# bacpop/ska.rust

Measured on AMD Instinct MI355X. Metric: genomes/sec ska build+align, 1 000x5 Mbp k=31; bit-exact vs CPU, higher is better.
Workload: dtype u64

## Files before the change

ska.rust_amd/csrc/skx_api.cpp:

```cpp
#include "skx_internal.h"
#include <algorithm>
#include <atomic>
#include <chrono>
#include <cmath>
#include <condition_variable>
#include <deque>
#include <cstdarg>
#include <cstddef>
#include <cstdio>
#include <cstring>
#include <map>
#include <memory>
#include <mutex>
#include <numeric>
#include <unordered_map>
#include <thread>
#include <cerrno>
#include <fcntl.h>
#include <sys/mman.h>
#include <sys/stat.h>
#include <unistd.h>

using namespace skx;

// ... 2482 lines not shown
{
    return skx_guarded([&]() -> int {
    skx_ctx *ctx = a->ctx; hipStream_t st = ctx->stream;
    SKX_HIP(hipSetDevice(ctx->device));
    const size_t S = a->names.size();
    if (a->pieces) {
        skx_pieces *pc = a->pieces;
        if (pc->sample_cells.size() != S) {
            DevBuf<unsigned long long> d; SKX_TRY(d.alloc(S)); SKX_TRY(d.zero(st));
            launch_pieces_cells(pc->data.p, pc->plen.p, pc->cap, (int)S, 1 << pc->logQ, d.p, st);
            std::vector<unsigned long long> h(S);
            SKX_HIP(hipMemcpyAsync(h.data(), d.p, S * 8, hipMemcpyDeviceToHost, st));
            SKX_HIP(hipStreamSynchronize(st));
            pc->sample_cells.assign(h.begin(), h.end());
        }
        for (size_t i = 0; i < S; i++) out[i] = (int64_t)pc->sample_cells[i];
        return SKX_OK;
    }
    if (a->lazy()) { for (size_t i = 0; i < S; i++) out[i] = (int64_t)a->lazy_dict->sample_size[i]; return SKX_OK; }
    DevBuf<unsigned long long> d; SKX_TRY(d.alloc(S)); SKX_TRY(d.zero(st));
    launch_row_nonmissing(a->matrix.p, a->pitch, (int)S, a->n_rows, d.p, st);
    std::vector<unsigned long long> h(S);
    SKX_HIP(hipMemcpyAsync(h.data(), d.p, S * 8, hipMemcpyDeviceToHost, st));
    SKX_HIP(hipStreamSynchronize(st));
    for (size_t i = 0; i < S; i++) out[i] = (int64_t)h[i];
    return SKX_OK;
    });
}

extern "C" int skx_array_pieces_info(skx_array *a, uint64_t *piece_bytes, uint64_t *row_blocks, uint32_t *ranks_per_block)
{
    return skx_guarded([&]() -> int {
    if (!a) { set_error("bad arguments"); return SKX_EINVAL; }
    if (piece_bytes) *piece_bytes = 0;
    if (row_blocks) *row_blocks = 0;
    if (ranks_per_block) *ranks_per_block = 0;
    const skx_pieces *pc = a->pieces;
    if (!pc) return SKX_OK;
    skx_ctx *ctx = a->ctx; hipStream_t st = ctx->stream;
    SKX_HIP(hipSetDevice(ctx->device));
    const uint64_t n = ((uint64_t)1 << pc->logQ) * a->names.size();
    std::vector<uint16_t> h(n);
    SKX_HIP(hipMemcpyAsync(h.data(), pc->plen.p, n * 2, hipMemcpyDeviceToHost, st));
    SKX_HIP(hipStreamSynchronize(st));
    uint64_t b = 0;
    for (uint16_t v : h) b += ((uint64_t)v + 31) / 32 * 16;
    if (piece_bytes) *piece_bytes = b;
    if (row_blocks) *row_blocks = (uint64_t)1 << pc->logQ;
    if (ranks_per_block) *ranks_per_block = pc->cap;
    return SKX_OK;
    });
}

static int array_compact(skx_array *a, DevBuf<uint8_t> &keep, DevBuf<uint64_t> &pos, uint64_t kept, int mask_ambig, bool vcount_from_unambig,
                         bool keys_follow)
{
    skx_ctx *ctx = a->ctx; hipStream_t st = ctx->stream;
    const uint64_t U = a->n_rows; const size_t S = a->names.size();
    const bool filter_ambig_as_missing = vcount_from_unambig;
    if (kept == U && !mask_ambig) {
        if (filter_ambig_as_missing && U) SKX_HIP(hipMemcpyAsync(a->vcount.p, a->unambig.p, U * 4, hipMemcpyDeviceToDevice, st));
        SKX_HIP(hipStreamSynchronize(st));
        return SKX_OK;
    }
    {
        StageTimer t(ctx, &ctx->tm.compact);
        const uint64_t np = pitch_for(kept);
        DevBuf<uint8_t> nm; DevBuf<uint32_t> p2, u2, m2, v2;
        SKX_TRY(nm.alloc((uint64_t)S * np)); SKX_TRY(p2.alloc(kept)); SKX_TRY(u2.alloc(kept)); SKX_TRY(m2.alloc(kept)); SKX_TRY(v2.alloc(kept));
        if (a->pieces) {
            PiecesRowsArgs pa = pieces_args(a);
            pa.out = nm.p; pa.pitch = np; pa.keep = keep.p; pa.kpos = pos.p; pa.mask_ambig = mask_ambig;
            KernelTimer kt(ctx, &ctx->tm.pieces_rows);
            launch_pieces_rows(pa, 1u << a->pieces->logQ, st);
        } else if (a->lazy()) {
            DevBuf<int> d_flag; SKX_TRY(d_flag.alloc(1)); SKX_TRY(d_flag.zero(st));
            AssembleArgs aa = lazy_args(a, d_flag.p);
            aa.matrix = nm.p; aa.pitch = np; aa.keep = keep.p; aa.kpos = pos.p; aa.mask_ambig = mask_ambig;
            { StageTimer t2(ctx, &ctx->tm.assemble); launch_assemble_lazy(a, aa, st, 2); }
            SKX_TRY(lazy_check_missing(a, d_flag));
        } else
            launch_compact_matrix(a->matrix.p, a->pitch, nm.p, np, (int)S, U, keep.p, pos.p, mask_ambig, st);
        launch_compact_u32(a->present.p, p2.p, U, keep.p, pos.p, st);
        launch_compact_u32(a->unambig.p, u2.p, U, keep.p, pos.p, st);
        launch_compact_u32(a->mask.p, m2.p, U, keep.p, pos.p, st);
        launch_compact_u32(filter_ambig_as_missing ? a->unambig.p : a->vcount.p, v2.p, U, keep.p, pos.p, st);
        if (mask_ambig) launch_mask_ambig_stats(m2.p, kept, st);
        if (a->n_kmers == U && keys_follow) {
            if (a->k <= 31) {
                DevBuf<uint64_t> k2; SKX_TRY(k2.alloc(kept));
                launch_compact_u64(a->keys.p, k2.p, U, keep.p, pos.p, st);
                a->keys = std::move(k2);
            } else if (a->host_keys.empty()) {
                DevBuf<uint64_t> k2; SKX_TRY(k2.alloc(kept * 2));
                launch_compact_u128(a->keys.p, k2.p, U, keep.p, pos.p, st);
                a->keys = std::move(k2);
            } else {
                std::vector<uint8_t> hkeep(U);
                SKX_HIP(hipMemcpyAsync(hkeep.data(), keep.p, U, hipMemcpyDeviceToHost, st));
                SKX_HIP(hipStreamSynchronize(st));
                std::vector<skx_key> nk; nk.reserve(kept);
                for (uint64_t i = 0; i < U; i++) if (hkeep[i] == 1) nk.push_back(a->host_keys[i]);
                a->host_keys.swap(nk);
            }
            a->n_kmers = kept;
        }
        SKX_HIP(hipStreamSynchronize(st));
        a->matrix = std::move(nm); a->present = std::move(p2); a->unambig = std::move(u2); a->mask = std::move(m2); a->vcount = std::move(v2);
        a->pitch = np; a->n_rows = kept;
        a->drop_lazy();
    }
    return SKX_OK;
}

extern "C" int skx_array_filter(skx_array *a, uint64_t min_count, int filter_ambig_as_missing, int filter_type, int mask_ambig,
                                int ignore_const_gaps, int update_kmers, int32_t *removed)
{
    return skx_guarded([&]() -> int {
    skx_ctx *ctx = a->ctx; hipStream_t st = ctx->stream;
    SKX_HIP(hipSetDevice(ctx->device));
    const uint64_t U = a->n_rows; const size_t S = a->names.size();
    SKX_TRY(array_lazy_stats(a));
    DevBuf<uint8_t> keep; DevBuf<uint64_t> pos;
    SKX_TRY(keep.alloc(U)); SKX_TRY(pos.alloc(U + 1));
    uint64_t kept = 0, silent = 0;
    {
        StageTimer t(ctx, &ctx->tm.filter);
        FilterArgs fa{a->vcount.p, a->present.p, a->unambig.p, a->mask.p, U, (uint32_t)(a->total_samples ? a->total_samples : S), min_count, filter_ambig_as_missing, filter_type, ignore_const_gaps, keep.p};
        launch_filter_flags(fa, st);
        DevBuf<uint32_t> sc_sums; DevBuf<uint64_t> sc_offs;
        SKX_TRY(sc_sums.alloc(scan_u8_blocks(U))); SKX_TRY(sc_offs.alloc(scan_u8_blocks(U) + 1));
        launch_scan_u8(keep.p, pos.p, U, sc_sums.p, sc_offs.p, st);
        SKX_HIP(hipMemcpyAsync(&kept, pos.p + U, 8, hipMemcpyDeviceToHost, st));
        if (filter_ambig_as_missing) {
            DevBuf<unsigned long long> d_sil; SKX_TRY(d_sil.alloc(1)); SKX_TRY(d_sil.zero(st));
            launch_count_u8(keep.p, U, 2, d_sil.p, st);
            unsigned long long s2 = 0;
            SKX_HIP(hipMemcpyAsync(&s2, d_sil.p, 8, hipMemcpyDeviceToHost, st));
            SKX_HIP(hipStreamSynchronize(st));
            silent = s2;
        }
        SKX_HIP(hipStreamSynchronize(st));
    }
    SKX_TRY(array_compact(a, keep, pos, kept, mask_ambig, filter_ambig_as_missing != 0, update_kmers || filter_ambig_as_missing));
    SKX_HIP(hipGetLastError());
    if (removed) *removed = (int32_t)(U - kept - silent);
    return SKX_OK;
    });
}


static int array_keep_rows(skx_array *a, DevBuf<uint8_t> &keep, uint64_t *removed)
{
    hipStream_t st = a->ctx->stream;
    const uint64_t U = a->n_rows;
    DevBuf<uint64_t> pos; SKX_TRY(pos.alloc(U + 1));
    uint64_t kept = 0;
    DevBuf<uint32_t> sc_sums; DevBuf<uint64_t> sc_offs;
    SKX_TRY(sc_sums.alloc(scan_u8_blocks(U))); SKX_TRY(sc_offs.alloc(scan_u8_blocks(U) + 1));
    launch_scan_u8(keep.p, pos.p, U, sc_sums.p, sc_offs.p, st);
// ... 473 lines not shown
```

ska.rust_amd/csrc/skx_api_io.cpp:

```cpp
#include "skx_internal.h"
#include "../../include/skx_host.h"
#include <algorithm>
#include <atomic>
#include <chrono>
#include <cmath>
#include <cstdio>
#include <cstring>
#include <memory>
#include <numeric>
#include <thread>
#include <unistd.h>
#include <fcntl.h>

using namespace skx;

extern "C" int skx_cov_histogram(skx_ctx *ctx, const char *fastq_fwd, const char *fastq_rev, int k, int rc, uint32_t *hist)
{
    return skx_guarded([&]() -> int {
    if (!ctx || !fastq_fwd || !fastq_rev || !hist) { set_error("bad arguments"); return SKX_EINVAL; }
    SKX_TRY(check_k(k));
    SKX_HIP(hipSetDevice(ctx->device));
    hipStream_t st = ctx->stream;
    HostStream hs[2];
    const char *files[2] = {fastq_fwd, fastq_rev};
// ... 599 lines not shown
            const uint64_t nb = (row_done * S) & ~7ull, left = have_hi - row_done * S;
            if (left) SKX_HIP(hipMemcpyAsync(d_cells[cur ^ 1].p + (row_done * S - nb), d_cells[cur].p + (row_done * S - base_cell), left, hipMemcpyDeviceToDevice, st));
        }
        SKX_HIP(hipStreamSynchronize(st));
        if (kept + gk > cap - 256) {
            const uint64_t ncap = pitch_for(std::max((kept + gk) * 2, cap * 2));
            DevBuf<uint8_t> nm; SKX_TRY(nm.alloc(S * ncap));
            if (kept) SKX_HIP(hipMemcpy2DAsync(nm.p, ncap, a->matrix.p, cap, kept, S, hipMemcpyDeviceToDevice, st));
            SKX_HIP(hipStreamSynchronize(st));
            a->matrix = std::move(nm); cap = ncap;
        }
        if (gk) launch_compact_rm(in, S, nr, keep.p + row_lo, pos.p, a->matrix.p, cap, kept, f->two_stage ? 0 : f->mask_ambig, st);
        kept += gk;
        row_lo = row_done; cur ^= 1;
        g0 = g1;
    }
    {
        const int wr = sf.walk_result();
        if (wr == SKF_NOT_TAKEN) { a->prealloc.reset(); a.reset(); return load_then_filter(ctx, path, f, out, removed, constant); }
        if (wr != SKX_OK) return wr;
    }
    int status = 0, bad = 0;
    SKX_HIP(hipMemcpyAsync(&status, d_status.p, 4, hipMemcpyDeviceToHost, st));
    SKX_HIP(hipMemcpyAsync(&bad, d_bad.p, 4, hipMemcpyDeviceToHost, st));
    SKX_HIP(hipStreamSynchronize(st));
    SKX_HIP(hipGetLastError());
    t_data.stop();
    if (status == 3) { tail.join(); a.reset(); return load_then_filter(ctx, path, f, out, removed, constant); }
    if (status) { set_error(status == 2 ? "skf: checksum mismatch" : "skf: corrupt snappy block"); return SKX_EFORMAT; }
    if (bad) { set_error("variants contain a byte outside -ACGTMRWSYKVHDBN (not supported on the device path)"); return SKX_EUNSUP; }
    tail.join();
    if (tail_rc != SKX_OK) { set_error("%s", tail_err.c_str()); return tail_rc; }
    PhaseTimer t_fin("load.counts_check_statistics");
    DevBuf<uint32_t> d_counts; SKX_TRY(d_counts.alloc(U));
    SKX_HIP(hipMemcpyAsync(d_counts.p, counts.data(), U * 4, hipMemcpyHostToDevice, st));
    if (!(f->filter_ambig_as_missing && !f->two_stage)) {
        SKX_TRY(d_status.zero(st));
        launch_differ_u32(d_counts.p, present.p, U, d_status.p, st);
        int differ = 0;
        SKX_HIP(hipMemcpyAsync(&differ, d_status.p, 4, hipMemcpyDeviceToHost, st));
        SKX_HIP(hipStreamSynchronize(st));
        if (differ) { a.reset(); return load_then_filter(ctx, path, f, out, removed, constant); }
    }
    unsigned long long n_silent = 0, n_const = 0;
    {
        DevBuf<unsigned long long> d_cnt; SKX_TRY(d_cnt.alloc(2)); SKX_TRY(d_cnt.zero(st));
        launch_count_u8(keep.p, U, 2, d_cnt.p, st); launch_count_u8(keep.p, U, 3, d_cnt.p + 1, st);
        unsigned long long h[2] = {0, 0};
        SKX_HIP(hipMemcpyAsync(h, d_cnt.p, 16, hipMemcpyDeviceToHost, st));
        DevBuf<uint64_t> gpos; DevBuf<uint32_t> s2; DevBuf<uint64_t> o2;
        SKX_TRY(gpos.alloc(U + 1)); SKX_TRY(s2.alloc(scan_u8_blocks(U) + 1)); SKX_TRY(o2.alloc(scan_u8_blocks(U) + 2));
        launch_scan_u8(keep.p, gpos.p, U, s2.p, o2.p, st);
        SKX_TRY(a->present.alloc(kept)); SKX_TRY(a->unambig.alloc(kept)); SKX_TRY(a->mask.alloc(kept)); SKX_TRY(a->vcount.alloc(kept));
        launch_compact_u32(present.p, a->present.p, U, keep.p, gpos.p, st);
        launch_compact_u32(unambig.p, a->unambig.p, U, keep.p, gpos.p, st);
        launch_compact_u32(mask.p, a->mask.p, U, keep.p, gpos.p, st);
        launch_compact_u32((f->filter_ambig_as_missing && !f->two_stage) ? unambig.p : d_counts.p, a->vcount.p, U, keep.p, gpos.p, st);
        if (f->mask_ambig && !f->two_stage) launch_mask_ambig_stats(a->mask.p, kept, st);
        SKX_HIP(hipStreamSynchronize(st));
        n_silent = h[0]; n_const = h[1];
    }
    SKX_HIP(hipGetLastError());
    a->k_bits = sf.m.k_bits; a->version = sf.m.version.empty() ? skx_version() : sf.m.version;
    a->n_rows = kept; a->pitch = cap;
    if (removed) *removed = (int64_t)(U - kept - n_silent - n_const);
    if (constant) *constant = (int64_t)n_const;
    rel.t = std::chrono::steady_clock::now(); rel.on = true;
    *out = a.release();
    return SKX_OK;
    });
}
```

ska.rust_amd/csrc/skx_append.hip:

```cpp
#include "skx_device.h"
#include <cstdlib>
#include <type_traits>

namespace skx {

typedef uint32_t u32x4 __attribute__((ext_vector_type(4)));
typedef const u32x4 __attribute__((address_space(1))) *g4_t;

#ifdef SKX_AP_PROF
__device__ unsigned long long g_ap_prof[16];
#define AP_PROF_START unsigned long long tprof = __builtin_readcyclecounter(), tacc[12] = {0, 0, 0, 0, 0, 0, 0, 0, 0, 0, 0, 0}
#define AP_PROF(i) do { const unsigned long long t_ = __builtin_readcyclecounter(); tacc[(i)] += t_ - tprof; tprof = t_; } while (0)
#define AP_PROF_FLUSH() do { for (int i_ = 0; i_ < 12; i_++) if (tacc[i_] && (i_ >= 6 || (threadIdx.x & 63) == 0)) atomicAdd(&g_ap_prof[i_], tacc[i_]); } while (0)
extern "C" void skx_debug_phase_prof(unsigned long long *out, int reset)
{
    unsigned long long h[16];
    (void)hipDeviceSynchronize();
    (void)hipMemcpyFromSymbol(h, HIP_SYMBOL(g_ap_prof), sizeof(h));
    for (int i = 0; i < 16; i++) out[i] = h[i];
    if (reset) { for (auto &x : h) x = 0; (void)hipMemcpyToSymbol(HIP_SYMBOL(g_ap_prof), h, sizeof(h)); }
}
#else
#define AP_PROF_START do { } while (0)
#define AP_PROF(i) do { } while (0)
// ... 594 lines not shown
    for (uint32_t p = threadIdx.x; p < nrows; p += 256) {
        const uint32_t pr = s_pr[p];
        o_present[r0 + p] = pr; o_vcount[r0 + p] = pr;
        o_unambig[r0 + p] = s_un[p]; o_mask[r0 + p] = s_mk[p];
    }
}
void launch_pieces_stats(const uint8_t *pieces, const uint16_t *plen, const uint16_t *perm, const uint32_t *nrank, const uint32_t *ncnt, const uint64_t *roff, uint32_t cap,
                         int n_samples, int n_blocks, uint32_t *present, uint32_t *unambig, uint32_t *mask, uint32_t *vcount, hipStream_t st)
{
    if (n_blocks <= 0) return;
    const unsigned gy = (cap / 32 + 255u) / 256u;
    static const int direct = knob("stats_direct") ? 1 : 0;
    const uint32_t stage = (cap + 63u) / 64u * 64u;
    hipLaunchKernelGGL(pieces_stats_kernel, dim3((unsigned)n_blocks, gy), dim3(256), (size_t)stage * 6, st, pieces, plen, perm, nrank, ncnt, roff, cap, n_samples, present, unambig, mask, vcount,
                       direct, stage);
}
__global__ __launch_bounds__(256) void pieces_cells_kernel(const uint8_t *pieces, const uint16_t *plen, uint32_t cap, int S, unsigned long long *out)
{
    const uint64_t j = blockIdx.x;
    const int lane = threadIdx.x & 63;
    for (int s = blockIdx.y * 4 + (threadIdx.x >> 6); s < S; s += gridDim.y * 4) {
        const uint32_t pl = plen[j * (uint64_t)S + s];
        const uint32_t *src = reinterpret_cast<const uint32_t *>(pieces + (j * (uint64_t)S + s) * (cap / 2));
        uint32_t c = 0;
        for (uint32_t i = lane; i < (pl + 7u) / 8u; i += 64) { const uint32_t x = src[i]; uint32_t t = x | (x >> 1); t |= t >> 2; c += (uint32_t)__popc(t & 0x11111111u); }
#pragma unroll
        for (int dd = 32; dd >= 1; dd >>= 1) c += __shfl_xor(c, dd, 64);
        if (lane == 0 && c) atomicAdd(&out[s], (unsigned long long)c);
    }
}
void launch_pieces_cells(const uint8_t *pieces, const uint16_t *plen, uint32_t cap, int n_samples, int n_blocks, unsigned long long *out, hipStream_t st)
{
    if (n_blocks <= 0 || n_samples <= 0) return;
    unsigned gy = (unsigned)((n_samples + 3) / 4); if (gy > 16) gy = 16;
    hipLaunchKernelGGL(pieces_cells_kernel, dim3((unsigned)n_blocks, gy), dim3(256), 0, st, pieces, plen, cap, n_samples, out);
}
__global__ __launch_bounds__(256) void region_totals_kernel(const uint32_t *raw, int logB, unsigned long long *out)
{
    __shared__ unsigned long long s_sum[256];
    const uint64_t B = 1ull << logB;
    unsigned long long t = 0;
    for (uint64_t b = threadIdx.x; b < B; b += 256) t += raw[(uint64_t)blockIdx.x * B + b];
    s_sum[threadIdx.x] = t;
    __syncthreads();
    for (int d = 128; d >= 1; d >>= 1) { if ((int)threadIdx.x < d) s_sum[threadIdx.x] += s_sum[threadIdx.x + d]; __syncthreads(); }
    if (threadIdx.x == 0) out[blockIdx.x] = s_sum[0];
}
void launch_region_totals(const uint32_t *raw, int n_samples, int logB, unsigned long long *out, hipStream_t st)
{
    if (n_samples > 0) hipLaunchKernelGGL(region_totals_kernel, dim3((unsigned)n_samples), dim3(256), 0, st, raw, logB, out);
}

constexpr int PR_WAVES = 8;
__device__ static inline uint32_t ap_iupac4(uint32_t m)
{
    const uint32_t idx = m & 0x07070707u;
    const uint32_t lo = __builtin_amdgcn_perm(0x48595754u, 0x4D43412Du, idx);
    const uint32_t hi = __builtin_amdgcn_perm(0x4E42444Bu, 0x56535247u, idx);
    const uint32_t sel = ((m >> 3) & 0x01010101u) * 0xFFu;
    return (hi & sel) | (lo & ~sel);
}
template <bool KEPT>
__global__ __launch_bounds__(64 * PR_WAVES) void pieces_rows_kernel(PiecesRowsArgs a)
{
    extern __shared__ __attribute__((aligned(16))) unsigned char s_raw[];
    const uint32_t cap = a.cap;
    uint16_t *s_src = reinterpret_cast<uint16_t *>(s_raw);
    uint32_t *s_piece = reinterpret_cast<uint32_t *>(s_raw + (((size_t)cap + 16) * 2 + 15) / 16 * 16);
    const uint64_t j = (uint64_t)blockIdx.x + a.j_base;
    const uint32_t n = a.ncnt[j];
    if (n == 0) return;
    const uint64_t r0 = a.roff[j];
    const uint64_t k0 = KEPT ? a.kpos[r0] : 0;
    const uint32_t nout = KEPT ? (uint32_t)(a.kpos[r0 + n] - k0) : n;
    if (nout == 0) return;
    const int tid = threadIdx.x, lane = tid & 63, wv = tid >> 6;
    const uint64_t ocol = KEPT ? k0 : r0 - a.col_base;
    const uint32_t shift = (uint32_t)(ocol & 3u);
    const uint32_t ndw = (nout + shift + 3u) / 4u;
    const uint16_t *pj = a.perm + j * (uint64_t)cap;
    const uint32_t nr = a.nrank[j];
    const int S = a.n_samples;
    const int s_lo = blockIdx.y * a.samples_per_wg, s_hi = s_lo + a.samples_per_wg < S ? s_lo + a.samples_per_wg : S;
    uint32_t *pc = s_piece + (size_t)wv * (cap / 8 + 4);
    const unsigned char *pcb = reinterpret_cast<const unsigned char *>(pc);
    const uint32_t nrw = (nr + 7u) / 8u;
    if (lane < 4) pc[cap / 8 + lane] = 0u;
    for (uint32_t t0 = 0; t0 < nout + shift; t0 += cap) {
        for (uint32_t i = tid; i < cap + 16u; i += blockDim.x) s_src[i] = (uint16_t)cap;
        __syncthreads();
        for (uint32_t r = tid; r < nr; r += blockDim.x) {
            const uint32_t p = pj[r];
            if (p == 0xFFFFu || p >= n) continue;
            uint32_t sc;
            if (!KEPT) sc = shift + p;
            else if (a.keep[r0 + p] == 1) sc = shift + (uint32_t)(a.kpos[r0 + p] - k0);
            else continue;
            if (sc >= t0 && sc < t0 + cap) s_src[sc - t0] = (uint16_t)r;
        }
        __syncthreads();
        const uint32_t v_lo = t0 / 4u, v_hi = (t0 + cap) / 4u < ndw ? (t0 + cap) / 4u : ndw;
        for (int s = s_lo + wv; s < s_hi; s += PR_WAVES) {
            const uint32_t pl = a.plen[j * (uint64_t)S + s];
            const uint32_t plw = (pl + 7u) / 8u;
            const uint32_t *src = reinterpret_cast<const uint32_t *>(a.pieces + (j * (uint64_t)S + s) * (cap / 2));
            {
                const uint4 *src4 = reinterpret_cast<const uint4 *>(src);
                uint4 *pc4 = reinterpret_cast<uint4 *>(pc);
                for (uint32_t i = lane; i < (nrw + 3u) / 4u; i += 64) {
                    uint4 x = 4u * i < plw ? src4[i] : make_uint4(0u, 0u, 0u, 0u);
                    if (4u * i + 1u >= plw) x.y = 0u;
                    if (4u * i + 2u >= plw) x.z = 0u;
                    if (4u * i + 3u >= plw) x.w = 0u;
                    pc4[i] = x;
                }
            }
            __builtin_amdgcn_wave_barrier();
            unsigned char *dst = a.out + (uint64_t)s * a.pitch + (ocol - shift);
            for (uint32_t v = v_lo + lane; v < v_hi; v += 64) {
                const uint2 rr = *reinterpret_cast<const uint2 *>(s_src + 4u * (v - v_lo));
                const uint32_t ra = rr.x & 0xFFFFu, rb = rr.x >> 16, rc = rr.y & 0xFFFFu, rd = rr.y >> 16;
                const uint32_t na = ((uint32_t)pcb[ra >> 1] >> ((ra & 1u) * 4u)) & 15u, nb = ((uint32_t)pcb[rb >> 1] >> ((rb & 1u) * 4u)) & 15u;
                const uint32_t nc = ((uint32_t)pcb[rc >> 1] >> ((rc & 1u) * 4u)) & 15u, nd = ((uint32_t)pcb[rd >> 1] >> ((rd & 1u) * 4u)) & 15u;
                uint32_t m = na | (nb << 8) | (nc << 16) | (nd << 24);
                uint32_t word = ap_iupac4(m);
                if (a.mask_ambig) {
                    const uint32_t y = m & (m - ((m | (m >> 1) | (m >> 2) | (m >> 3)) & 0x01010101u));
                    const uint32_t amb = ((y | (y >> 1) | (y >> 2) | (y >> 3)) & 0x01010101u) * 0xFFu;
                    word = (word & ~amb) | (0x4E4E4E4Eu & amb);
                }
                const bool head = v == 0 && shift != 0, tail = v == ndw - 1 && ((nout + shift) & 3u) != 0;
                if (!head && !tail) *reinterpret_cast<uint32_t *>(dst + 4u * v) = word;
                else {
#pragma unroll
                    for (int b = 0; b < 4; b++) { const int c = (int)(4u * v + b) - (int)shift; if (c >= 0 && (uint32_t)c < nout) dst[4u * v + b] = (unsigned char)(word >> (8 * b)); }
                }
            }
            __builtin_amdgcn_wave_barrier();
        }
        __syncthreads();
    }
}
void launch_pieces_rows(const PiecesRowsArgs &a, uint32_t n_blocks, hipStream_t st)
{
    if (!n_blocks || a.n_samples <= 0) return;
    PiecesRowsArgs b = a;
    int spw = a.n_samples;
    while (spw > PR_WAVES * 4 && (uint64_t)n_blocks * ((a.n_samples + spw - 1) / spw) < 8192) spw = (spw + 1) / 2;
    b.samples_per_wg = spw;
    const unsigned gy = (unsigned)((a.n_samples + spw - 1) / spw);
    const size_t lds = (((size_t)a.cap + 16) * 2 + 15) / 16 * 16 + (size_t)PR_WAVES * (a.cap / 8 + 4) * 4;
    if (a.keep) {
        (void)hipFuncSetAttribute((const void *)pieces_rows_kernel<true>, hipFuncAttributeMaxDynamicSharedMemorySize, (int)lds);
        hipLaunchKernelGGL(pieces_rows_kernel<true>, dim3(n_blocks, gy), dim3(64 * PR_WAVES), lds, st, b);
    } else {
        (void)hipFuncSetAttribute((const void *)pieces_rows_kernel<false>, hipFuncAttributeMaxDynamicSharedMemorySize, (int)lds);
        hipLaunchKernelGGL(pieces_rows_kernel<false>, dim3(n_blocks, gy), dim3(64 * PR_WAVES), lds, st, b);
    }
}

}

#include "skx_append_wide.inc"
```

ska.rust_amd/csrc/skx_device.h:

```cpp
#pragma once
#include <hip/hip_runtime.h>
#include <stdint.h>

namespace skx {

long knob(const char *name, long absent = 0);
int extract_tile_bases(int logB);
constexpr int MAX_LOGB = 13;
constexpr uint64_t EMPTY64 = ~0ull;

struct HashParams {
    int bits;
    int hb;
    uint32_t hmask;
    uint32_t c[4];
};
HashParams make_hash_params(int k);
__host__ __device__ inline uint32_t hround(uint32_t v, uint32_t c, int hb) { return (v * c) >> (32 - hb); }
__host__ __device__ inline void hmix_halves(uint32_t &L, uint32_t &R, const HashParams &p)
{
    L ^= hround(R, p.c[0], p.hb); R ^= hround(L, p.c[1], p.hb);
}
__host__ __device__ inline uint64_t hmix(uint64_t x, const HashParams &p)
{
// ... 85 lines not shown
    uint64_t pitch;
    uint32_t *col_present;
    uint32_t *col_unambig;
    uint32_t *col_mask;
    uint32_t max_rows;
    int *missing;
    uint32_t j_base = 0;
    uint64_t col_base = 0;
    const uint8_t *keep = nullptr; const uint64_t *kpos = nullptr;
    int mask_ambig = 0;
};
void launch_assemble(const AssembleArgs &a, hipStream_t st, int mode = 0, uint32_t n_blocks = 0);
bool union_side_ok(const DictView &d, int logN, uint32_t stride);
void launch_union_side(const DictView &d, int logN, uint64_t *stage, uint32_t stride, uint32_t *ncnt, uint32_t table_slots, int *overflow,
                       uint16_t *side, uint16_t *perm, hipStream_t st);
void launch_assemble_side(const AssembleArgs &a, const uint16_t *side, const uint16_t *perm, hipStream_t st, bool wide = false);
void launch_compose_perm(const uint64_t *l_stage, uint32_t l_stride, const uint32_t *l_ncnt, const uint16_t *l_perm, int l_logN, const uint64_t *g_stage,
                         uint32_t g_stride, const uint32_t *g_ncnt, const uint64_t *g_roff, int g_logN, int bits, uint16_t *g_perm, uint32_t *g_n,
                         uint64_t *g_base, uint32_t *g_max, int *bad, hipStream_t st);
void launch_union_side_wide(const DictView &d, int logN, u128 *stage, uint32_t stride, uint32_t *ncnt, uint32_t table_slots, int *overflow,
                            uint16_t *side, uint16_t *perm, hipStream_t st);

constexpr uint32_t APPEND_MAX_CAP = 6016, APPEND_MAX_SLOTS = 8192;
struct AppendArgs {
    const uint64_t *words; const uint64_t *off; const uint32_t *raw;
    int n_samples, logB, bits, logQ;
    uint32_t nslots, cap;
    uint8_t *pieces; uint16_t *plen; uint16_t *perm; uint32_t *nrank;
    uint64_t *stage; uint32_t stride; uint32_t *ncnt;
    unsigned long long *probe;
    int *overflow;
    uint32_t rounds = 1;
    int *bar = nullptr;
};
bool append_ok(int bits, int logB, int logQ, uint32_t region_cap, uint32_t nslots, uint32_t cap);
void launch_append(const AppendArgs &a, uint32_t region_cap, hipStream_t st);
void launch_append_probe(const AppendArgs &a, uint32_t region_cap, unsigned blocks, hipStream_t st);
constexpr uint32_t APPEND_WIDE_MAX_CAP = 3072, APPEND_WIDE_MAX_SLOTS = 4096;
bool append_wide_ok(int bits, int logB, int logQ, uint32_t nslots, uint32_t cap);
void launch_append_wide(const AppendArgs &a, hipStream_t st);
void launch_append_wide_probe(const AppendArgs &a, unsigned blocks, hipStream_t st);
void launch_pieces_stats(const uint8_t *pieces, const uint16_t *plen, const uint16_t *perm, const uint32_t *nrank, const uint32_t *ncnt, const uint64_t *roff, uint32_t cap,
                         int n_samples, int n_blocks, uint32_t *present, uint32_t *unambig, uint32_t *mask, uint32_t *vcount, hipStream_t st);
void launch_pieces_cells(const uint8_t *pieces, const uint16_t *plen, uint32_t cap, int n_samples, int n_blocks, unsigned long long *out, hipStream_t st);
void launch_region_totals(const uint32_t *raw, int n_samples, int logB, unsigned long long *out, hipStream_t st);
struct PiecesRowsArgs {
    const uint8_t *pieces; const uint16_t *plen; const uint16_t *perm; const uint32_t *nrank; uint32_t cap; int n_samples;
    const uint32_t *ncnt; const uint64_t *roff;
    uint8_t *out; uint64_t pitch;
    uint32_t j_base = 0; uint64_t col_base = 0;
    const uint8_t *keep = nullptr; const uint64_t *kpos = nullptr;
    int mask_ambig = 0;
    int samples_per_wg = 0;
};
void launch_pieces_rows(const PiecesRowsArgs &a, uint32_t n_blocks, hipStream_t st);

void launch_gather_keys(const uint64_t *stage, uint32_t stride, const uint32_t *ncnt, const uint64_t *roff, int n_sub,
                        uint64_t *out, int unhash, HashParams hp, hipStream_t st);
void launch_hash_keys(const uint64_t *keys, uint64_t *words, uint64_t n, HashParams hp, hipStream_t st);
void launch_keys_cbor(const uint64_t *words, uint64_t n, HashParams hp, uint8_t *out, int *short_key, hipStream_t st);
void launch_unhash_dict(const uint64_t *words, uint64_t n, uint64_t *keys, uint8_t *bases, HashParams hp, hipStream_t st);

void launch_col_stats(const uint8_t *matrix, uint64_t pitch, int n_samples, uint64_t n_cols, uint32_t *present,
                      uint32_t *unambig, uint32_t *mask, int *bad_byte, hipStream_t st);
struct FilterArgs {
    const uint32_t *vcount, *present, *unambig, *mask; uint64_t n_cols; uint32_t n_samples;
    uint64_t min_count; int ambig_as_missing, filter_type, ignore_const_gaps;
    uint8_t *keep;
    int two_stage = 0;
};
void launch_filter_flags(const FilterArgs &a, hipStream_t st);
void launch_row_stats_rm(const uint8_t *cells, uint64_t S, uint64_t nr, uint32_t *present, uint32_t *unambig, uint32_t *mask, int *bad_byte, hipStream_t st);
void launch_compact_rm(const uint8_t *cells, uint64_t S, uint64_t nr, const uint8_t *keep, const uint64_t *pos, uint8_t *out, uint64_t pitch,
                       uint64_t col0, int mask_ambig, hipStream_t st);
uint64_t scan_u8_blocks(uint64_t n);
void launch_scan_u8(const uint8_t *flags, uint64_t *pos, uint64_t n, uint32_t *sums, uint64_t *offs, hipStream_t st);
void launch_compact_matrix(const uint8_t *in, uint64_t in_pitch, uint8_t *out, uint64_t out_pitch, int n_samples,
                           uint64_t n_cols, const uint8_t *keep, const uint64_t *pos, int mask_ambig, hipStream_t st);
void launch_compact_u32(const uint32_t *in, uint32_t *out, uint64_t n, const uint8_t *keep, const uint64_t *pos, hipStream_t st);
void launch_compact_u64(const uint64_t *in, uint64_t *out, uint64_t n, const uint8_t *keep, const uint64_t *pos, hipStream_t st);
void launch_compact_u128(const uint64_t *in, uint64_t *out, uint64_t n, const uint8_t *keep, const uint64_t *pos, hipStream_t st);
void launch_mask_ambig_stats(uint32_t *mask, uint64_t n, hipStream_t st);
void launch_count_u8(const uint8_t *v, uint64_t n, uint8_t value, unsigned long long *out, hipStream_t st);
void launch_differ_u32(const uint32_t *a, const uint32_t *b, uint64_t n, int *flag, hipStream_t st);
void launch_transpose(const uint8_t *in, uint64_t in_pitch, uint64_t rows, uint64_t cols, uint8_t *out, uint64_t out_pitch,
                      hipStream_t st);
struct SnapChunk { uint64_t src_off, uoff; uint32_t src_len, ulen, crc, compressed; };
constexpr uint32_t SKF_SLOT = 8 + 65536;
int launch_skf_decode_cells(int device, const uint8_t *src, const SnapChunk *chunks, uint32_t n_chunks, uint64_t upos, uint64_t uend,
                            uint8_t *scratch , uint8_t *cells, uint64_t base_cell, int *status, hipStream_t st);
int launch_skf_encode_cells(int device, const uint8_t *cells, uint64_t base_cell, uint64_t upos, uint64_t uoff0, uint32_t n_chunks,
                            uint8_t *slots, uint32_t *sizes, hipStream_t st);
void launch_skf_gather(const uint8_t *slots, const uint32_t *sizes, const uint64_t *off, uint32_t n_chunks, uint8_t *dense, hipStream_t st);
void launch_row_nonmissing(const uint8_t *matrix, uint64_t pitch, int n_samples, uint64_t n_cols, unsigned long long *out,
                           hipStream_t st);

void launch_build_planes(const uint8_t *matrix, uint64_t pitch, int n_samples, uint64_t n_cols, uint64_t *planes, uint64_t wpr, int filt,
                         hipStream_t st);
void launch_keep_bits(const uint8_t *keep, const uint64_t *pos, uint64_t n, uint64_t *keep_bits, uint64_t *gpos, hipStream_t st);
void launch_split_keep(const uint8_t *keep, const uint32_t *col_mask, uint64_t n, uint8_t *clean, uint8_t *dirty, hipStream_t st, int mode = 0);
void launch_split_keep_from_dirty(uint8_t *dirty, uint64_t n, uint8_t *clean, hipStream_t st);
void launch_build_planes_keep(const uint8_t *matrix, uint64_t pitch, int n_samples, uint64_t n_cols, const uint64_t *keep_bits, const uint64_t *gpos,
                              uint64_t *planes, uint64_t wpr, int filt, hipStream_t st, uint32_t *first_group, uint64_t kept);
constexpr int DIST_NCOUNT = 16;
int launch_pair_counts(const uint64_t *planes, int n_samples, uint64_t words_per_row, int filt_ambig,
                       unsigned long long *out, hipStream_t st, int i_lo = 0, int i_hi = 0);

void launch_hist_wide(const ExtractArgs &a, hipStream_t st);
void launch_scatter_wide(const ExtractArgs &a, hipStream_t st);
int extract_tile_bases_wide();
void launch_dedupe_wide(u128 *words, const uint64_t *off, const uint32_t *raw, uint32_t *ucnt, uint64_t n_regions, uint32_t cap,
                        int rem_bits, int *overflow, uint16_t *sidx, int sb, hipStream_t st);
void launch_union_wide(const DictView &d, int logN, u128 *stage, uint32_t stride, uint32_t *ncnt, uint32_t table_slots, int *overflow,
                       hipStream_t st);
void launch_union_probe_wide(const DictView &d, int logP, int probe, uint32_t *cnt, uint32_t table_slots, int *overflow, hipStream_t st);
void launch_assemble_wide(const AssembleArgs &a, hipStream_t st, int mode = 0, uint32_t n_blocks = 0);
void launch_gather_keys_wide(const u128 *stage, uint32_t stride, const uint32_t *ncnt, const uint64_t *roff, int n_sub, u128 *out,
                             hipStream_t st);

uint64_t fasta_parse_tiles(uint64_t len);
#ifdef __HIPCC__
__device__ static inline void planes_bytes16(const uint64_t *groups, uint64_t t, uint64_t len, uint32_t sw[4], uint32_t qw[4])
{
    const uint64_t p0 = t * 16;
    const uint64_t *g = groups + (t >> 2) * 5;
    const int sh = (int)(t & 3) * 16;
    const uint32_t lo = (uint32_t)(g[0] >> sh) & 0xFFFFu, hi = (uint32_t)(g[1] >> sh) & 0xFFFFu, bad = (uint32_t)(g[2] >> sh) & 0xFFFFu,
                   nl = (uint32_t)(g[3] >> sh) & 0xFFFFu, qb = (uint32_t)(g[4] >> sh) & 0xFFFFu;
#pragma unroll
    for (int i = 0; i < 4; i++) {
        uint32_t x = 0, y = 0;
#pragma unroll
// ... 46 lines not shown
```

ska.rust_amd/csrc/skx_device2.inc:

```
namespace skx {

__device__ static inline uint32_t set_code(uint32_t b)
{
    switch (b) {
    case '-': return 0;
    case 'A': return 1;  case 'C': return 2;  case 'M': return 3;  case 'T': return 4;
    case 'W': return 5;  case 'Y': return 6;  case 'H': return 7;  case 'G': return 8;
    case 'R': return 9;  case 'S': return 10; case 'V': return 11; case 'K': return 12;
    case 'D': return 13; case 'B': return 14; case 'N': return 15;
    default: return 0xFF;
    }
}

__global__ __launch_bounds__(256) void col_stats_kernel(const uint8_t *matrix, uint64_t pitch, int n_samples, uint64_t n_cols,
                                                        uint32_t *present, uint32_t *unambig, uint32_t *mask, int *bad_byte)
{
    const uint64_t c0 = ((uint64_t)blockIdx.x * blockDim.x + threadIdx.x) * 4;
    if (c0 >= n_cols) return;
    uint32_t p[4] = {0, 0, 0, 0}, u[4] = {0, 0, 0, 0}, m[4] = {0, 0, 0, 0};
    int bad = 0;
    for (int s = 0; s < n_samples; s++) {
        const uint32_t x = *reinterpret_cast<const uint32_t *>(matrix + (uint64_t)s * pitch + c0);
#pragma unroll
        for (int i = 0; i < 4; i++) {
// ... 65 lines not shown
        const uint32_t kw[4] = {k4.x, k4.y, k4.z, k4.w};
#pragma unroll
        for (int i = 0; i < 16; i++) kf |= (uint32_t)(((kw[i >> 2] >> (8 * (i & 3))) & 0xFFu) == 1u) << i;
    } else if (c < n_cols)
        for (int i = 0; i < 16; i++) kf |= (uint32_t)(c + i < n_cols && keep[c + i] == 1) << i;
    uint32_t total;
    const uint32_t lofs = block_excl_scan(__popc(kf), s_tmp, &total);
    if (total == 0) return;
    const uint64_t cblk = (uint64_t)blockIdx.x * blockDim.x * 16;
    const uint64_t p0 = pos[cblk < n_cols ? cblk : n_cols - 1];
    const uint32_t shift = (uint32_t)(p0 & 15u);
    const uint32_t stride = (4096 + 32 + 15) & ~15u;
    const int s0 = blockIdx.y * CMP_ROWS, s1 = s0 + CMP_ROWS < n_samples ? s0 + CMP_ROWS : n_samples;
    if (kf) {
        const uint8_t *src = in + (uint64_t)s0 * in_pitch + c;
#pragma unroll 2
        for (int s = s0; s < s1; s++, src += in_pitch) {
            const uint4 x4 = *reinterpret_cast<const uint4 *>(src);
            const uint32_t xw[4] = {x4.x, x4.y, x4.z, x4.w};
            unsigned char *d = s_buf + (size_t)(s - s0) * stride + shift + lofs;
            uint32_t o = 0;
#pragma unroll
            for (int i = 0; i < 16; i++)
                if ((kf >> i) & 1u) { const uint8_t b = (uint8_t)(xw[i >> 2] >> (8 * (i & 3))); d[o++] = mask_ambig ? mask_ambig_byte(b) : b; }
        }
    }
    __syncthreads();
    const int lane = threadIdx.x & 63, wv = threadIdx.x >> 6;
    const uint32_t head = (16u - shift) & 15u, h = head < total ? head : total, body = (total - h) / 16u, done = h + body * 16u;
    for (int s = s0 + wv; s < s1; s += 4) {
        const unsigned char *row = s_buf + (size_t)(s - s0) * stride + shift;
        uint8_t *dst = out + (uint64_t)s * out_pitch + p0;
        if ((uint32_t)lane < h) dst[lane] = row[lane];
        for (uint32_t v = lane; v < body; v += 64) *reinterpret_cast<uint4 *>(dst + h + 16u * v) = *reinterpret_cast<const uint4 *>(row + h + 16u * v);
        if (done + lane < total) dst[done + lane] = row[done + lane];
    }
}
void launch_compact_matrix(const uint8_t *in, uint64_t in_pitch, uint8_t *out, uint64_t out_pitch, int n_samples, uint64_t n_cols,
                           const uint8_t *keep, const uint64_t *pos, int mask_ambig, hipStream_t st)
{
    if (!n_cols || !n_samples) return;
    const uint64_t groups = (n_cols + 15) / 16;
    const size_t lds = (size_t)CMP_ROWS * ((4096 + 32 + 15) & ~15u);
    (void)hipFuncSetAttribute((const void *)compact_matrix_kernel, hipFuncAttributeMaxDynamicSharedMemorySize, (int)lds);
    hipLaunchKernelGGL(compact_matrix_kernel, dim3((unsigned)((groups + 255) / 256), (unsigned)((n_samples + CMP_ROWS - 1) / CMP_ROWS)), dim3(256),
                       lds, st, in, in_pitch, out, out_pitch, n_samples, n_cols, keep, pos, mask_ambig);
}
template <typename T>
__global__ void compact_vec_kernel(const T *in, T *out, uint64_t n, const uint8_t *keep, const uint64_t *pos)
{
    for (uint64_t c = (uint64_t)blockIdx.x * blockDim.x + threadIdx.x; c < n; c += (uint64_t)gridDim.x * blockDim.x)
        if (keep[c] == 1) out[pos[c]] = in[c];
}
void launch_compact_u32(const uint32_t *in, uint32_t *out, uint64_t n, const uint8_t *keep, const uint64_t *pos, hipStream_t st)
{
    if (!n) return;
    uint64_t g = (n + 255) / 256; if (g > 8192) g = 8192;
    hipLaunchKernelGGL(compact_vec_kernel<uint32_t>, dim3((unsigned)g), dim3(256), 0, st, in, out, n, keep, pos);
}
void launch_compact_u64(const uint64_t *in, uint64_t *out, uint64_t n, const uint8_t *keep, const uint64_t *pos, hipStream_t st)
{
    if (!n) return;
    uint64_t g = (n + 255) / 256; if (g > 8192) g = 8192;
    hipLaunchKernelGGL(compact_vec_kernel<uint64_t>, dim3((unsigned)g), dim3(256), 0, st, in, out, n, keep, pos);
}
struct alignas(16) pair64 { uint64_t a, b; };
void launch_compact_u128(const uint64_t *in, uint64_t *out, uint64_t n, const uint8_t *keep, const uint64_t *pos, hipStream_t st)
{
    if (!n) return;
    uint64_t g = (n + 255) / 256; if (g > 8192) g = 8192;
    hipLaunchKernelGGL(compact_vec_kernel<pair64>, dim3((unsigned)g), dim3(256), 0, st, (const pair64 *)in, (pair64 *)out, n, keep, pos);
}
__global__ void mask_ambig_stats_kernel(uint32_t *mask, uint64_t n)
{
    const uint64_t c = (uint64_t)blockIdx.x * blockDim.x + threadIdx.x;
    if (c >= n) return;
    const uint32_t acgt = (1u << 1) | (1u << 2) | (1u << 4) | (1u << 8);
    uint32_t m = mask[c];
    if (m & ~acgt) m = (m & acgt) | (1u << 15);
    mask[c] = m;
}
void launch_mask_ambig_stats(uint32_t *mask, uint64_t n, hipStream_t st)
{
    if (!n) return;
    hipLaunchKernelGGL(mask_ambig_stats_kernel, dim3((unsigned)((n + 255) / 256)), dim3(256), 0, st, mask, n);
}

__global__ __launch_bounds__(256) void row_stats_rm_kernel(const uint8_t *cells, uint64_t S, uint64_t nr, uint32_t *present, uint32_t *unambig,
                                                           uint32_t *mask, int *bad_byte)
{
    __shared__ uint8_t s_lut[256];
    s_lut[threadIdx.x] = (uint8_t)set_code(threadIdx.x);
    __syncthreads();
    const int lane = threadIdx.x & 63;
    const uint64_t waves = (uint64_t)gridDim.x * 4;
    for (uint64_t r = (uint64_t)blockIdx.x * 4 + (threadIdx.x >> 6); r < nr; r += waves) {
        const int64_t b = (int64_t)(r * S), e = b + (int64_t)S;
        const int64_t skew = (int64_t)(((uintptr_t)cells + (uintptr_t)b) & 3u);
        uint32_t p = 0, u = 0, m = 0; bool bad = false;
        for (int64_t a = b - skew + 4 * lane; a < e; a += 256) {
            const uint32_t x = *reinterpret_cast<const uint32_t *>(cells + a);
#pragma unroll
            for (int i = 0; i < 4; i++) {
                const int64_t q = a + i;
                if (q < b || q >= e) continue;
                const uint32_t code = s_lut[(x >> (8 * i)) & 0xFFu];
                if (code == 0xFF) { bad = true; continue; }
                if (code) { p++; u += (code & (code - 1)) == 0; m |= 1u << code; }
            }
        }
        for (int d = 32; d; d >>= 1) { p += __shfl_down(p, d, 64); u += __shfl_down(u, d, 64); m |= __shfl_down(m, d, 64); }
// ... 639 lines not shown
```

Before: 29050.

## Fuse per-column stats compaction and trim kept-row piece loads to highest used rank

Four separate compaction launches for present/unambig/mask/vcount are merged into one kernel that reads keep and pos once. In the kept-rows pieces kernel, the keep/kpos lookups are batched four at a time, and a block-wide max of the used row rank limits how many packed piece words each wave loads into LDS. Debug counters and knobs for counting piece loads and forcing full loads are also added. The trade-off is an extra atomic and barrier per tile, plus some unused instrumentation branches.

```diff
diff --git a/ska.rust_amd/csrc/skx_api.cpp b/ska.rust_amd/csrc/skx_api.cpp
--- a/ska.rust_amd/csrc/skx_api.cpp
+++ b/ska.rust_amd/csrc/skx_api.cpp
@@ -2558,6 +2558,7 @@
     });
 }
 
+extern "C" int skx_debug_kept_piece_loads(unsigned long long *out, int reset);
 static int array_compact(skx_array *a, DevBuf<uint8_t> &keep, DevBuf<uint64_t> &pos, uint64_t kept, int mask_ambig, bool vcount_from_unambig,
                          bool keys_follow)
 {
@@ -2587,10 +2588,7 @@
             SKX_TRY(lazy_check_missing(a, d_flag));
         } else
             launch_compact_matrix(a->matrix.p, a->pitch, nm.p, np, (int)S, U, keep.p, pos.p, mask_ambig, st);
-        launch_compact_u32(a->present.p, p2.p, U, keep.p, pos.p, st);
-        launch_compact_u32(a->unambig.p, u2.p, U, keep.p, pos.p, st);
-        launch_compact_u32(a->mask.p, m2.p, U, keep.p, pos.p, st);
-        launch_compact_u32(filter_ambig_as_missing ? a->unambig.p : a->vcount.p, v2.p, U, keep.p, pos.p, st);
+        launch_compact_stats(a->present.p, a->unambig.p, a->mask.p, filter_ambig_as_missing ? a->unambig.p : a->vcount.p, p2.p, u2.p, m2.p, v2.p, U, keep.p, pos.p, st);
         if (mask_ambig) launch_mask_ambig_stats(m2.p, kept, st);
         if (a->n_kmers == U && keys_follow) {
             if (a->k <= 31) {
@@ -2612,6 +2610,11 @@
             a->n_kmers = kept;
         }
         SKX_HIP(hipStreamSynchronize(st));
+        if (a->pieces && getenv("SKX_DEBUG") && knob("kept_count_ranks")) {
+            unsigned long long c[3] = {0, 0, 0};
+            if (skx_debug_kept_piece_loads(c, 0) == 0)
+                fprintf(stderr, "[skx] kept rows: %llu piece loads, %llu column passes, %llu beyond a block's first (counted since the process began)\n", c[0], c[1], c[2]);
+        }
         a->matrix = std::move(nm); a->present = std::move(p2); a->unambig = std::move(u2); a->mask = std::move(m2); a->vcount = std::move(v2);
         a->pitch = np; a->n_rows = kept;
         a->drop_lazy();
diff --git a/ska.rust_amd/csrc/skx_api_io.cpp b/ska.rust_amd/csrc/skx_api_io.cpp
--- a/ska.rust_amd/csrc/skx_api_io.cpp
+++ b/ska.rust_amd/csrc/skx_api_io.cpp
@@ -675,10 +675,8 @@
         SKX_TRY(gpos.alloc(U + 1)); SKX_TRY(s2.alloc(scan_u8_blocks(U) + 1)); SKX_TRY(o2.alloc(scan_u8_blocks(U) + 2));
         launch_scan_u8(keep.p, gpos.p, U, s2.p, o2.p, st);
         SKX_TRY(a->present.alloc(kept)); SKX_TRY(a->unambig.alloc(kept)); SKX_TRY(a->mask.alloc(kept)); SKX_TRY(a->vcount.alloc(kept));
-        launch_compact_u32(present.p, a->present.p, U, keep.p, gpos.p, st);
-        launch_compact_u32(unambig.p, a->unambig.p, U, keep.p, gpos.p, st);
-        launch_compact_u32(mask.p, a->mask.p, U, keep.p, gpos.p, st);
-        launch_compact_u32((f->filter_ambig_as_missing && !f->two_stage) ? unambig.p : d_counts.p, a->vcount.p, U, keep.p, gpos.p, st);
+        launch_compact_stats(present.p, unambig.p, mask.p, (f->filter_ambig_as_missing && !f->two_stage) ? unambig.p : d_counts.p, a->present.p, a->unambig.p, a->mask.p,
+                             a->vcount.p, U, keep.p, gpos.p, st);
         if (f->mask_ambig && !f->two_stage) launch_mask_ambig_stats(a->mask.p, kept, st);
         SKX_HIP(hipStreamSynchronize(st));
         n_silent = h[0]; n_const = h[1];
diff --git a/ska.rust_amd/csrc/skx_append.hip b/ska.rust_amd/csrc/skx_append.hip
--- a/ska.rust_amd/csrc/skx_append.hip
+++ b/ska.rust_amd/csrc/skx_append.hip
@@ -670,6 +670,16 @@
 }
 
 constexpr int PR_WAVES = 8;
+__device__ unsigned long long g_kept_counts[3];
+extern "C" int skx_debug_kept_piece_loads(unsigned long long *out , int reset)
+{
+    unsigned long long h[3] = {0, 0, 0};
+    hipError_t e = hipDeviceSynchronize();
+    if (e == hipSuccess) e = hipMemcpyFromSymbol(h, HIP_SYMBOL(g_kept_counts), sizeof(h));
+    if (e == hipSuccess && out) for (int i = 0; i < 3; i++) out[i] = h[i];
+    if (e == hipSuccess && reset) { for (auto &x : h) x = 0; e = hipMemcpyToSymbol(HIP_SYMBOL(g_kept_counts), h, sizeof(h)); }
+    return (int)e;
+}
 __device__ static inline uint32_t ap_iupac4(uint32_t m)
 {
     const uint32_t idx = m & 0x07070707u;
@@ -678,10 +688,42 @@
     const uint32_t sel = ((m >> 3) & 0x01010101u) * 0xFFu;
     return (hi & sel) | (lo & ~sel);
 }
+__device__ static inline uint4 pr_trim(uint4 x, uint32_t i, uint32_t plw)
+{
+    if (4u * i >= plw) x.x = 0u;
+    if (4u * i + 1u >= plw) x.y = 0u;
+    if (4u * i + 2u >= plw) x.z = 0u;
+    if (4u * i + 3u >= plw) x.w = 0u;
+    return x;
+}
+__device__ static inline void pr_gather(const PiecesRowsArgs &a, const uint16_t *s_src, const unsigned char *pcb, unsigned char *dst, uint32_t v_lo, uint32_t v_hi,
+                                        uint32_t ndw, uint32_t nout, uint32_t shift, int lane)
+{
+    for (uint32_t v = v_lo + lane; v < v_hi; v += 64) {
+        const uint2 rr = *reinterpret_cast<const uint2 *>(s_src + 4u * (v - v_lo));
+        const uint32_t ra = rr.x & 0xFFFFu, rb = rr.x >> 16, rc = rr.y & 0xFFFFu, rd = rr.y >> 16;
+        const uint32_t na = ((uint32_t)pcb[ra >> 1] >> ((ra & 1u) * 4u)) & 15u, nb = ((uint32_t)pcb[rb >> 1] >> ((rb & 1u) * 4u)) & 15u;
+        const uint32_t nc = ((uint32_t)pcb[rc >> 1] >> ((rc & 1u) * 4u)) & 15u, nd = ((uint32_t)pcb[rd >> 1] >> ((rd & 1u) * 4u)) & 15u;
+        uint32_t m = na | (nb << 8) | (nc << 16) | (nd << 24);
+        uint32_t word = ap_iupac4(m);
+        if (a.mask_ambig) {
+            const uint32_t y = m & (m - ((m | (m >> 1) | (m >> 2) | (m >> 3)) & 0x01010101u));
+            const uint32_t amb = ((y | (y >> 1) | (y >> 2) | (y >> 3)) & 0x01010101u) * 0xFFu;
+            word = (word & ~amb) | (0x4E4E4E4Eu & amb);
+        }
+        const bool head = v == 0 && shift != 0, tail = v == ndw - 1 && ((nout + shift) & 3u) != 0;
+        if (!head && !tail) *reinterpret_cast<uint32_t *>(dst + 4u * v) = word;
+        else {
+#pragma unroll
+            for (int b = 0; b < 4; b++) { const int c = (int)(4u * v + b) - (int)shift; if (c >= 0 && (uint32_t)c < nout) dst[4u * v + b] = (unsigned char)(word >> (8 * b)); }
+        }
+    }
+}
 template <bool KEPT>
 __global__ __launch_bounds__(64 * PR_WAVES) void pieces_rows_kernel(PiecesRowsArgs a)
 {
     extern __shared__ __attribute__((aligned(16))) unsigned char s_raw[];
+    __shared__ uint32_t s_rmax;
     const uint32_t cap = a.cap;
     uint16_t *s_src = reinterpret_cast<uint16_t *>(s_raw);
     uint32_t *s_piece = reinterpret_cast<uint32_t *>(s_raw + (((size_t)cap + 16) * 2 + 15) / 16 * 16);
@@ -702,62 +744,63 @@
     const int s_lo = blockIdx.y * a.samples_per_wg, s_hi = s_lo + a.samples_per_wg < S ? s_lo + a.samples_per_wg : S;
     uint32_t *pc = s_piece + (size_t)wv * (cap / 8 + 4);
     const unsigned char *pcb = reinterpret_cast<const unsigned char *>(pc);
-    const uint32_t nrw = (nr + 7u) / 8u;
     if (lane < 4) pc[cap / 8 + lane] = 0u;
+    unsigned long long n_loads = 0;
     for (uint32_t t0 = 0; t0 < nout + shift; t0 += cap) {
         for (uint32_t i = tid; i < cap + 16u; i += blockDim.x) s_src[i] = (uint16_t)cap;
+        if (KEPT && tid == 0) s_rmax = 0u;
         __syncthreads();
-        for (uint32_t r = tid; r < nr; r += blockDim.x) {
-            const uint32_t p = pj[r];
-            if (p == 0xFFFFu || p >= n) continue;
-            uint32_t sc;
-            if (!KEPT) sc = shift + p;
-            else if (a.keep[r0 + p] == 1) sc = shift + (uint32_t)(a.kpos[r0 + p] - k0);
-            else continue;
-            if (sc >= t0 && sc < t0 + cap) s_src[sc - t0] = (uint16_t)r;
-        }
-        __syncthreads();
+        uint32_t rmax = nr;
+        if (!KEPT) {
+            for (uint32_t r = tid; r < nr; r += blockDim.x) {
+                const uint32_t p = pj[r];
+                if (p == 0xFFFFu || p >= n) continue;
+                const uint32_t sc = shift + p;
+                if (sc >= t0 && sc < t0 + cap) s_src[sc - t0] = (uint16_t)r;
+            }
+            __syncthreads();
+        } else {
+            uint32_t hi = 0;
+            for (uint32_t rb = tid; rb < nr; rb += 4u * blockDim.x) {
+                uint32_t p[4]; uint8_t kp[4]; uint64_t kq[4];
+#pragma unroll
+                for (int i = 0; i < 4; i++) { const uint32_t r = rb + (uint32_t)i * blockDim.x; p[i] = pj[r < nr ? r : 0u]; if (r >= nr) p[i] = 0xFFFFu; }
+#pragma unroll
+                for (int i = 0; i < 4; i++) { const bool ok = p[i] != 0xFFFFu && p[i] < n; if (!ok) p[i] = 0u; kp[i] = a.keep[r0 + p[i]]; if (!ok) kp[i] = 0; }
+#pragma unroll
+                for (int i = 0; i < 4; i++) kq[i] = a.kpos[r0 + p[i]];
+#pragma unroll
+                for (int i = 0; i < 4; i++) {
+                    if (kp[i] != 1) continue;
+                    const uint32_t r = rb + (uint32_t)i * blockDim.x, sc = shift + (uint32_t)(kq[i] - k0);
+                    if (sc >= t0 && sc < t0 + cap) { s_src[sc - t0] = (uint16_t)r; hi = r + 1u; }
+                }
+            }
+#pragma unroll
+            for (int dd = 32; dd >= 1; dd >>= 1) { const uint32_t o = (uint32_t)__shfl_xor((int)hi, dd, 64); hi = o > hi ? o : hi; }
+            if (lane == 0 && hi) atomicMax(&s_rmax, hi);
+            __syncthreads();
+            if (!a.full_pieces) rmax = s_rmax;
+            if (a.count && tid == 0) { atomicAdd(a.count + 1, 1ull); if (t0) atomicAdd(a.count + 2, 1ull); }
+        }
+        const uint32_t nrw = (rmax + 7u) / 8u;
+        const uint32_t nq = (nrw + 3u) / 4u;
         const uint32_t v_lo = t0 / 4u, v_hi = (t0 + cap) / 4u < ndw ? (t0 + cap) / 4u : ndw;
+        uint4 *pc4 = reinterpret_cast<uint4 *>(pc);
         for (int s = s_lo + wv; s < s_hi; s += PR_WAVES) {
             const uint32_t pl = a.plen[j * (uint64_t)S + s];
             const uint32_t plw = (pl + 7u) / 8u;
-            const uint32_t *src = reinterpret_cast<const uint32_t *>(a.pieces + (j * (uint64_t)S + s) * (cap / 2));
-            {
-                const uint4 *src4 = reinterpret_cast<const uint4 *>(src);
-                uint4 *pc4 = reinterpret_cast<uint4 *>(pc);
-                for (uint32_t i = lane; i < (nrw + 3u) / 4u; i += 64) {
-                    uint4 x = 4u * i < plw ? src4[i] : make_uint4(0u, 0u, 0u, 0u);
-                    if (4u * i + 1u >= plw) x.y = 0u;
-                    if (4u * i + 2u >= plw) x.z = 0u;
-                    if (4u * i + 3u >= plw) x.w = 0u;
-                    pc4[i] = x;
-                }
-            }
+            const uint4 *src4 = reinterpret_cast<const uint4 *>(a.pieces + (j * (uint64_t)S + s) * (cap / 2));
+            for (uint32_t i = lane; i < nq; i += 64)
+                pc4[i] = pr_trim(4u * i < plw ? src4[i] : make_uint4(0u, 0u, 0u, 0u), i, plw);
+            if (KEPT && a.count) n_loads += ((plw < nrw ? plw : nrw) + 3u) / 4u;
             __builtin_amdgcn_wave_barrier();
-            unsigned char *dst = a.out + (uint64_t)s * a.pitch + (ocol - shift);
-            for (uint32_t v = v_lo + lane; v < v_hi; v += 64) {
-                const uint2 rr = *reinterpret_cast<const uint2 *>(s_src + 4u * (v - v_lo));
-                const uint32_t ra = rr.x & 0xFFFFu, rb = rr.x >> 16, rc = rr.y & 0xFFFFu, rd = rr.y >> 16;
-                const uint32_t na = ((uint32_t)pcb[ra >> 1] >> ((ra & 1u) * 4u)) & 15u, nb = ((uint32_t)pcb[rb >> 1] >> ((rb & 1u) * 4u)) & 15u;
-                const uint32_t nc = ((uint32_t)pcb[rc >> 1] >> ((rc & 1u) * 4u)) & 15u, nd = ((uint32_t)pcb[rd >> 1] >> ((rd & 1u) * 4u)) & 15u;
-                uint32_t m = na | (nb << 8) | (nc << 16) | (nd << 24);
-                uint32_t word = ap_iupac4(m);
-                if (a.mask_ambig) {
-                    const uint32_t y = m & (m - ((m | (m >> 1) | (m >> 2) | (m >> 3)) & 0x01010101u));
-                    const uint32_t amb = ((y | (y >> 1) | (y >> 2) | (y >> 3)) & 0x01010101u) * 0xFFu;
-                    word = (word & ~amb) | (0x4E4E4E4Eu & amb);
-                }
-                const bool head = v == 0 && shift != 0, tail = v == ndw - 1 && ((nout + shift) & 3u) != 0;
-                if (!head && !tail) *reinterpret_cast<uint32_t *>(dst + 4u * v) = word;
-                else {
-#pragma unroll
-                    for (int b = 0; b < 4; b++) { const int c = (int)(4u * v + b) - (int)shift; if (c >= 0 && (uint32_t)c < nout) dst[4u * v + b] = (unsigned char)(word >> (8 * b)); }
-                }
-            }
+            pr_gather(a, s_src, pcb, a.out + (uint64_t)s * a.pitch + (ocol - shift), v_lo, v_hi, ndw, nout, shift, lane);
             __builtin_amdgcn_wave_barrier();
         }
         __syncthreads();
     }
+    if (KEPT && a.count && lane == 0 && n_loads) atomicAdd(a.count, n_loads);
 }
 void launch_pieces_rows(const PiecesRowsArgs &a, uint32_t n_blocks, hipStream_t st)
 {
@@ -769,6 +812,12 @@
     const unsigned gy = (unsigned)((a.n_samples + spw - 1) / spw);
     const size_t lds = (((size_t)a.cap + 16) * 2 + 15) / 16 * 16 + (size_t)PR_WAVES * (a.cap / 8 + 4) * 4;
     if (a.keep) {
+        b.full_pieces = knob("kept_full_pieces") ? 1 : 0;
+        b.count = nullptr;
+        if (knob("kept_count_ranks") && hipGetSymbolAddress((void **)&b.count, HIP_SYMBOL(g_kept_counts)) != hipSuccess) {
+            b.count = nullptr;
+            fprintf(stderr, "[skx] kept_count_ranks: no address for the counters, nothing is counted\n");
+        }
         (void)hipFuncSetAttribute((const void *)pieces_rows_kernel<true>, hipFuncAttributeMaxDynamicSharedMemorySize, (int)lds);
         hipLaunchKernelGGL(pieces_rows_kernel<true>, dim3(n_blocks, gy), dim3(64 * PR_WAVES), lds, st, b);
     } else {
diff --git a/ska.rust_amd/csrc/skx_device.h b/ska.rust_amd/csrc/skx_device.h
--- a/ska.rust_amd/csrc/skx_device.h
+++ b/ska.rust_amd/csrc/skx_device.h
@@ -161,6 +161,7 @@
     const uint8_t *keep = nullptr; const uint64_t *kpos = nullptr;
     int mask_ambig = 0;
     int samples_per_wg = 0;
+    int full_pieces = 0; unsigned long long *count = nullptr;
 };
 void launch_pieces_rows(const PiecesRowsArgs &a, uint32_t n_blocks, hipStream_t st);
 
@@ -186,7 +187,8 @@
 void launch_scan_u8(const uint8_t *flags, uint64_t *pos, uint64_t n, uint32_t *sums, uint64_t *offs, hipStream_t st);
 void launch_compact_matrix(const uint8_t *in, uint64_t in_pitch, uint8_t *out, uint64_t out_pitch, int n_samples,
                            uint64_t n_cols, const uint8_t *keep, const uint64_t *pos, int mask_ambig, hipStream_t st);
-void launch_compact_u32(const uint32_t *in, uint32_t *out, uint64_t n, const uint8_t *keep, const uint64_t *pos, hipStream_t st);
+void launch_compact_stats(const uint32_t *in_p, const uint32_t *in_u, const uint32_t *in_m, const uint32_t *in_v, uint32_t *out_p, uint32_t *out_u, uint32_t *out_m,
+                          uint32_t *out_v, uint64_t n, const uint8_t *keep, const uint64_t *pos, hipStream_t st);
 void launch_compact_u64(const uint64_t *in, uint64_t *out, uint64_t n, const uint8_t *keep, const uint64_t *pos, hipStream_t st);
 void launch_compact_u128(const uint64_t *in, uint64_t *out, uint64_t n, const uint8_t *keep, const uint64_t *pos, hipStream_t st);
 void launch_mask_ambig_stats(uint32_t *mask, uint64_t n, hipStream_t st);
diff --git a/ska.rust_amd/csrc/skx_device2.inc b/ska.rust_amd/csrc/skx_device2.inc
--- a/ska.rust_amd/csrc/skx_device2.inc
+++ b/ska.rust_amd/csrc/skx_device2.inc
@@ -141,11 +141,22 @@
     for (uint64_t c = (uint64_t)blockIdx.x * blockDim.x + threadIdx.x; c < n; c += (uint64_t)gridDim.x * blockDim.x)
         if (keep[c] == 1) out[pos[c]] = in[c];
 }
-void launch_compact_u32(const uint32_t *in, uint32_t *out, uint64_t n, const uint8_t *keep, const uint64_t *pos, hipStream_t st)
+__global__ void compact_stats_kernel(const uint32_t *in_p, const uint32_t *in_u, const uint32_t *in_m, const uint32_t *in_v, uint32_t *out_p, uint32_t *out_u,
+                                     uint32_t *out_m, uint32_t *out_v, uint64_t n, const uint8_t *keep, const uint64_t *pos)
+{
+    for (uint64_t c = (uint64_t)blockIdx.x * blockDim.x + threadIdx.x; c < n; c += (uint64_t)gridDim.x * blockDim.x) {
+        if (keep[c] != 1) continue;
+        const uint64_t o = pos[c];
+        const uint32_t p = in_p[c], u = in_u[c], m = in_m[c], v = in_v[c];
+        out_p[o] = p; out_u[o] = u; out_m[o] = m; out_v[o] = v;
+    }
+}
+void launch_compact_stats(const uint32_t *in_p, const uint32_t *in_u, const uint32_t *in_m, const uint32_t *in_v, uint32_t *out_p, uint32_t *out_u, uint32_t *out_m,
+                          uint32_t *out_v, uint64_t n, const uint8_t *keep, const uint64_t *pos, hipStream_t st)
 {
     if (!n) return;
     uint64_t g = (n + 255) / 256; if (g > 8192) g = 8192;
-    hipLaunchKernelGGL(compact_vec_kernel<uint32_t>, dim3((unsigned)g), dim3(256), 0, st, in, out, n, keep, pos);
+    hipLaunchKernelGGL(compact_stats_kernel, dim3((unsigned)g), dim3(256), 0, st, in_p, in_u, in_m, in_v, out_p, out_u, out_m, out_v, n, keep, pos);
 }
 void launch_compact_u64(const uint64_t *in, uint64_t *out, uint64_t n, const uint8_t *keep, const uint64_t *pos, hipStream_t st)
 {
```

Result: no change. 29220, median of 4 (+0.6%).
